# martenlienen/generative-turbulence

Hardware: AMD Instinct MI355X
Metric: U-Net fwd+bwd voxels/sec (DDPM training step, 192x64x48x4) (higher is better)
Workload: dtype bf16

## Files before the change

### generative-turbulence_amd/csrc/tdx_conv3.h

```cpp
#pragma once
#include "tdx_common.h"

struct Conv3Geom {
    int B;
    int Xi, Yi, Zi;
    int Xo, Yo, Zo;
    int off;
};

bool conv3_mfma_supported(int C1, int C2, int Cout);
bool conv3_mfma_f32_supported(int C1, int C2, int Cout);
static inline int conv3_layout_kc(int dtype, int K, int N) {
    if (dtype == 1 || dtype == 3) return conv3_mfma_supported(K, 0, N) ? 16 : 0;
    return conv3_mfma_f32_supported(K, 0, N) ? 8 : 0;
}
static inline bool conv3_uses_mfma_layout(int dtype, int K, int N) { return (dtype == 1 || dtype == 3) && conv3_mfma_supported(K, 0, N); }
bool conv3_mfma_split_supported(int C1, int C2, int Cout);

struct Conv3Ext {
    int ld1, ld2;
    const void* init;
    bool init_shared;
};

struct Conv3Call {
    const void* x1; int C1;
    const void* x2; int C2;
    const void* wp;
    const float* bias;
    void* y;
    int B, X, Y, Z, N;
    bool zero_pad;
    double* gn_acc;
    void* d1; int D1; void* d2;
    const void* a1; const void* a2;
    hipStream_t st;
    int fmt;
    const Conv3Ext* ext;
    const int* slabs_beyond;
    bool hf() const { return fmt == TDX_F16; }
    Conv3Geom geom() const { return Conv3Geom{B, X, Y, Z, X, Y, Z, 0}; }
};

struct SmallGeom {
    int B;
    int Ev[3];
    int Es[3];
    int off;
    int clamp;
    int nbg;
    int xs;
    int gx;
    int Ix, Iy, Iz;
    int K, N;
    int per_split;
    int nsplit;
};
struct Conv3SmallPlan {
    SmallGeom g;
    size_t lds;
    int mtw;
};

struct Conv3Route {
    int fmt, family, status;
    int ring_depth;
    Conv3SmallPlan small;
};
Conv3Route conv3_route(int dtype, int impl, int C1, int C2, int N, int B, int X, int Y, int Z, bool data_gradient);

int conv3_mfma_launch(const Conv3Call& c);
int conv3_mfma_split_launch(const Conv3Call& c);
int conv3_mfma_f32_launch(const Conv3Call& c);
int conv3_direct_launch(const Conv3Call& c);
int conv3_fold_launch(const Conv3Call& c);

int conv3_ring_depth(int C1, int C2, int N, int B, int X, int Y, int Z, bool data_gradient);
int conv3_ring_launch(const Conv3Call& c, int depth);

bool conv3_small_plan(Conv3SmallPlan& p, int C1, int C2, int N, int B, int X, int Y, int Z, bool data_gradient, bool split);
int conv3_small_launch(const Conv3Call& c, const Conv3SmallPlan& p);

struct Conv3WgradCall {
    const void* x1; int C1;
    const void* x2; int C2;
    const void* dy;
    float* dwp;
    float* dbias;
    int B, X, Y, Z, Cout;
    hipStream_t st;
    float* slabs; int max_slabs; int* nslab;
    bool hf;
};
bool tdx_deterministic();
static inline float* conv3_wgrad_merge(const Conv3WgradCall& c, int& nsplit, int64_t& slab_stride) {
    if (tdx_deterministic() && c.slabs != nullptr && nsplit > c.max_slabs) nsplit = c.max_slabs > 0 ? c.max_slabs : 1;
    const bool use_slabs = c.slabs != nullptr && nsplit <= c.max_slabs;
    slab_stride = use_slabs ? (int64_t)27 * (c.C1 + c.C2) * c.Cout : 0;
    if (c.nslab) *c.nslab = use_slabs ? nsplit : 0;
    return use_slabs ? c.slabs : c.dwp;
}
// ... 30 lines not shown
```

### generative-turbulence_amd/csrc/tdx_conv3_entry.hip

```cpp
#include "tdx_common.h"
#include "tdx_conv3.h"
#include <stdlib.h>
#include <algorithm>

int tdx_persistent_cus() {
    const char* env = getenv("TDX_PERSISTENT_CUS");
    int n = env ? atoi(env) : 256;
    n = n < 8 ? 8 : (n > 256 ? 256 : n);
    return n & ~7;
}
static void* g_scratch = nullptr;
static size_t g_scratch_bytes = 0;
void* tdx_scratch_ptr() { return g_scratch; }
size_t tdx_scratch_bytes() { return g_scratch_bytes; }
extern "C" int tdx_set_scratch(void* ptr, size_t bytes) {
    if (ptr != nullptr && bytes < 64) return TDX_EINVAL;
    g_scratch = ptr;
    g_scratch_bytes = ptr ? bytes : 0;
    return TDX_OK;
}

Conv3Route conv3_route(int dtype, int impl, int C1, int C2, int N, int B, int X, int Y, int Z, bool data_gradient) {
    Conv3Route r;
    r.fmt = dtype; r.family = TDX_KERNEL_DIRECT; r.status = TDX_OK; r.ring_depth = 0;
// ... 90 lines not shown
    if (!conv3_mfma_supported(C1, 0, Cout)) return TDX_ESHAPE;
    const bool det = tdx_deterministic();
    const Conv3Ext ext = {ld1, 0, init, init_shared != 0};
    Conv3Call c = conv3_fwd_call(x1, C1, nullptr, 0, wf, bias, y, B, X, Y, Z, Cout, dtype, stream);
    c.ext = &ext;
    c.gn_acc = (stats && !det) ? (double*)gn_workspace : nullptr;
    if (c.gn_acc && !clean) {
        int e = tdx_zero_async(c.gn_acc, (size_t)TDX_GN_REPLICAS * B * Cout * 2 * sizeof(double), c.st);
        if (e != TDX_OK) return e;
    }
    int rc = conv3_mfma_launch(c);
    if (rc != TDX_OK || !stats) return rc;
    if (det) return gn_stats_launch(y, stats, B, (int64_t)X * Y * Z, Cout, G, eps, dtype, gn_workspace, clean, c.st);
    return gn_finalize_launch(c.gn_acc, stats, B, Cout, G, (int64_t)X * Y * Z, eps, TDX_GN_REPLICAS, c.st);
}

extern "C" size_t tdx_conv3_bwd_data_workspace_bytes(int B, int X, int Y, int Z, int Cin, int dtype, int impl) {
    (void)impl;
    const size_t padded = (size_t)B * (X + 2) * (Y + 2) * (Z + 2) * Cin * (tdx_is_h16(dtype) ? 2 : 4);
    const size_t shell = conv3_shell_buffer_bytes(B, X, Y, Z, Cin);
    return (padded > shell ? padded : shell) + 256;
}

static int conv3_bwd_data_impl(const void* dy, const void* wb, void* dx1, int C1, void* dx2, int C2, const void* add1,
                               const void* add2, int B, int X, int Y, int Z, int Cout, int dtype, int impl,
                               void* workspace, void* stream) {
    TDX_CHECK_ARG(dy && wb && dx1 && workspace && B > 0 && X > 0 && Y > 0 && Z > 0 && C1 > 0 && C2 >= 0 && Cout > 0);
    TDX_CHECK_ARG(C2 == 0 || dx2);
    const int Cin = C1 + C2;
    if ((C1 % 8) || (C2 % 8) || (Cout % 8)) return TDX_ESHAPE;
    const Conv3Route r = conv3_route(dtype, impl, Cout, 0, Cin, B, X, Y, Z, true);
    if (r.status != TDX_OK) return r.status;
    Conv3Call c = {};
    c.x1 = dy; c.C1 = Cout; c.wp = wb;
    c.B = B; c.X = X; c.Y = Y; c.Z = Z; c.N = Cin;
    c.zero_pad = true;
    c.d1 = dx1; c.D1 = C1; c.d2 = dx2; c.a1 = add1; c.a2 = add2;
    c.st = as_stream(stream); c.fmt = r.fmt;
    if (r.family == TDX_KERNEL_DIRECT) c.y = workspace;
    int rc = conv3_launch(c, r);
    if (rc != TDX_OK || r.family == TDX_KERNEL_SMALL) return rc;
    if (r.family == TDX_KERNEL_DIRECT) return conv3_fold_launch(c);
    const int shell_mode = r.fmt == TDX_F16 ? 3 : (r.fmt == TDX_F32_SPLIT ? 2 : (r.fmt == TDX_F32 ? 1 : 0));
    return conv3_shell_launch(dy, wb, dx1, C1, dx2, B, X, Y, Z, Cout, Cin, shell_mode, c.st, workspace);
}

extern "C" int tdx_conv3_bwd_data(const void* dy, const void* wb, void* dx1, int C1, void* dx2, int C2,
                                  int accumulate, int B, int X, int Y, int Z, int Cout, int dtype, int impl,
                                  void* workspace, void* stream) {
    return conv3_bwd_data_impl(dy, wb, dx1, C1, dx2, C2, accumulate ? dx1 : nullptr, accumulate ? dx2 : nullptr, B, X, Y, Z,
                               Cout, dtype, impl, workspace, stream);
}

extern "C" int tdx_conv3_bwd_data_add(const void* dy, const void* wb, void* dx1, int C1, void* dx2, int C2,
                                      const void* add1, const void* add2, int B, int X, int Y, int Z, int Cout, int dtype,
                                      int impl, void* workspace, void* stream) {
    return conv3_bwd_data_impl(dy, wb, dx1, C1, dx2, C2, add1, add2, B, X, Y, Z, Cout, dtype, impl, workspace, stream);
}

#define W3_MAX_SLABS 8
static int w3_slab_capacity(int Cin, int Cout) {
    const int64_t c = ((int64_t)1 << 19) / ((int64_t)Cin * Cout);
    return (int)(c < W3_MAX_SLABS ? W3_MAX_SLABS : (c > 512 ? 512 : c));
}
extern "C" size_t tdx_conv3_bwd_weight_workspace_bytes(int Cin, int Cout, int impl) {
    (void)impl;
    return (size_t)(1 + w3_slab_capacity(Cin, Cout)) * 27 * Cin * Cout * sizeof(float) + (size_t)Cout * sizeof(float) + 512;
}

struct Conv3WgradRoute {
    int (*launch)(const Conv3WgradCall&);
    bool f32;
    int status;
};
static Conv3WgradRoute conv3_wgrad_route(int dtype, int impl, int C1, int C2, int Cout) {
    if (dtype == TDX_F32 && impl == TDX_CONV_SPLIT && conv3_wgrad_mfma_split_supported(C1, C2, Cout))
        return {conv3_wgrad_mfma_split_launch, true, TDX_OK};
    if (dtype == TDX_F32 && impl != TDX_CONV_DIRECT && conv3_wgrad_mfma_f32_supported(C1, C2, Cout))
        return {conv3_wgrad_mfma_f32_launch, true, TDX_OK};
    if (impl == TDX_CONV_MFMA || (impl == TDX_CONV_AUTO && tdx_is_h16(dtype) && conv3_wgrad_mfma_supported(C1, C2, Cout))) {
// ... 45 lines not shown
```

### generative-turbulence_amd/csrc/tdx_conv3_ring.hip

```cpp
#include "tdx_common.h"
#include "tdx_conv3.h"
#include "tdx_conv3_epilogue.h"
#include <algorithm>

#define RG_HY 10
#define RG_SZ 12
#define RG_SZ4 6
#define RG_WSLOTS 3
#define RG_WAVES 8
#define RG_STEPS 14
#ifndef RG_DEFAULT_LOADERS
#define RG_DEFAULT_LOADERS 1
#endif

struct RingArgs {
    const bf16* x1; const bf16* x2; int C1, C2;
    const bf16* wp; const float* bias; bf16* y;
    int B, X, Y, Z, Cout;
    int nbx, nby, nbz, ntn;
    double* gn_acc;
    bf16* d1; bf16* d2; int D1; const bf16* a1; const bf16* a2;
    const void* zeros;
    unsigned long long* stamps;
};

__device__ __forceinline__ void rg_dma_off(const void* sbase, unsigned voff, unsigned lds) {
    lds = __builtin_amdgcn_readfirstlane(lds);
    unsigned keep;
    asm volatile("s_mov_b32 %0, m0\n\ts_mov_b32 m0, %3\n\ts_nop 0\n\tglobal_load_lds_dwordx4 %1, %2\n\ts_mov_b32 m0, %0"
                 : "=&s"(keep) : "v"(voff), "s"(sbase), "s"(lds) : "memory");
}
#define RG_VMCNT(n) asm volatile("s_waitcnt vmcnt(%0)" ::"n"(n) : "memory")

#ifdef RG_STAMPS
#define RG_NSTAMP 64
#define RG_T()                                                                                        \
    do {                                                                                              \
        if (ord >= RG_STAMP_B0 && ord < RG_STAMP_B0 + 2) {                                            \
            const unsigned long long t_ = __builtin_amdgcn_s_memtime();                               \
            if (lane == 0 && nst < RG_NSTAMP) sStamp[wave * RG_NSTAMP + nst] = t_;                    \
            ++nst;                                                                                    \
        }                                                                                             \
    } while (0)
#else
#define RG_T() do { } while (0)
#endif
// ... 4 lines not shown
    static constexpr int BN = NT * 32;
    static constexpr int MT = 4 / NT;
    static constexpr int XP = Z4 ? MT : MT / 2;
    static constexpr int BX = 8 * XP;
    static constexpr int BZ = Z4 ? 4 : 8;
    static constexpr int HZ = BZ + 2;
    static constexpr int SZ = Z4 ? RG_SZ4 : RG_SZ;
    static constexpr int ENT = Z4 ? (BX + 2) / 2 * RG_HY * RG_SZ
                                  : (BX + 2) * RG_HY * SZ;
    static constexpr int APIECES = (ENT + 63) / 64;
    static constexpr int ABUF = APIECES * 1024;
    static constexpr int BPW = (APIECES + IW - 1) / IW;
    static constexpr int WPIECES = 28 * BN * 16 / 1024;
    static constexpr int WSLOT = WPIECES * 1024;
    static constexpr int WPW = (WPIECES + IW - 1) / IW;
    static constexpr int TILE = 32 * BN * 2;
    static constexpr int CH = BN / 8;
    static constexpr int VPI = 64 / CH;
    static constexpr int NST = MT * (32 / VPI);
    static constexpr size_t LDS = (size_t)2 * ABUF + (size_t)RG_WSLOTS * WSLOT + (size_t)RG_WAVES * TILE + 1024  +
                                  64  + BN * 4  + (size_t)RG_WAVES * BN * 2 * 4 ;
};

template <int NT, bool ZP, int LW, bool HF, bool Z4>
__global__ void __launch_bounds__(512 + 64 * LW, LW ? 3 : 2) conv3_ring_kernel(RingArgs A) {
    typedef RingShape<NT, LW, Z4> S;
    typedef H16<HF> H;
    typedef typename H::T HT;
    constexpr int BN = S::BN, MT = S::MT, XP = S::XP, BPW = S::BPW, WPW = S::WPW, CH = S::CH, VPI = S::VPI, NST = S::NST;
    static_assert(LW > 0 || BPW + WPW < RG_STEPS, "one DMA instruction per K step");
    extern __shared__ __attribute__((aligned(1024))) unsigned char smem[];
    unsigned char* sA = smem;
    unsigned char* sW = sA + 2 * S::ABUF;
    unsigned char* sT = sW + RG_WSLOTS * S::WSLOT;
    unsigned char* sD = sT + RG_WAVES * S::TILE;
    unsigned char* sZ = sD + 1024;
    float* sBias = reinterpret_cast<float*>(sZ + 64);
    float* sRed = sBias + BN;
    const unsigned lds0 = (unsigned)(size_t)(__attribute__((address_space(3))) const void*)smem;
    const unsigned ldsA = lds0, ldsW = lds0 + 2 * S::ABUF, ldsD = ldsW + RG_WSLOTS * S::WSLOT + RG_WAVES * S::TILE;

    const int tid = threadIdx.x, lane = tid & 63;
    const int wave = __builtin_amdgcn_readfirstlane(tid >> 6);
    const int r = lane & 31, hh = lane >> 5;
    const bool loader = LW > 0 && wave >= RG_WAVES;
    const int iw = LW ? wave - RG_WAVES : wave;
#ifdef RG_STAMPS
    unsigned long long* sStamp = reinterpret_cast<unsigned long long*>(NT == 2 ? sRed : sRed + RG_WAVES * BN * 2);
    int nst = 0;
#endif

    const int hw = blockIdx.x, xcd = hw & 7, slot = hw >> 3;
    const int ntile = slot % A.ntn, kx = slot / A.ntn, KX = (int)(gridDim.x >> 3) / A.ntn;
    const int nbricks = A.B * A.nbx * A.nby * A.nbz;
    const int lo = xcd * (nbricks >> 3) + min(xcd, nbricks & 7), hi = lo + (nbricks >> 3) + (xcd < (nbricks & 7) ? 1 : 0);
    const int nmine = hi - lo > kx ? (hi - lo - kx + KX - 1) / KX : 0;
    if (nmine == 0) return;
    const int n0 = ntile * BN;
    const int Cin = A.C1 + A.C2, nun = Cin >> 3;
    const int YZ = A.Y * A.Z, V = A.X * YZ;

    if (tid < BN) sBias[tid] = A.bias ? A.bias[n0 + tid] : 0.f;
    if (tid < 16) reinterpret_cast<unsigned*>(sZ)[tid] = 0u;
    lds_barrier();

    int hxyz[BPW];
#pragma unroll
    for (int i = 0; i < BPW; ++i) {
        const int pi = min(max(iw, 0) * BPW + i, S::APIECES - 1);
        const int e = min(pi * 64 + lane, S::ENT - 1);
        int hx, hy, hz;
        if (Z4) {
            const int xp = e / (RG_HY * RG_SZ), rem = e - xp * (RG_HY * RG_SZ), q = rem % RG_SZ;
            hy = rem / RG_SZ; hx = 2 * xp + q / RG_SZ4; hz = q % RG_SZ4;
        } else {
            hx = e / (RG_HY * S::SZ);
            const int rem = e - hx * (RG_HY * S::SZ);
            hy = rem / S::SZ; hz = min(rem - hy * S::SZ, S::HZ - 1);
        }
        hxyz[i] = hx | (hy << 8) | (hz << 16);
    }
    unsigned wlane[WPW];
#pragma unroll
    for (int j = 0; j < WPW; ++j) {
        const int pj = min(max(iw, 0) * WPW + j, S::WPIECES - 1);
        const int e = pj * 64 + lane;
// ... 138 lines not shown
#endif
        }
        RG_VMCNT(0);
        return;
    }
    bool stores_behind = false;

    f32x16 acc[NT][MT];

    for (int ord = 0; ord < nmine; ++ord) {
        int b, o0, o1, o2;
        brick_coords(ord, b, o0, o1, o2);
#pragma unroll
        for (int nt = 0; nt < NT; ++nt)
#pragma unroll
            for (int j = 0; j < 4; ++j) {
                const float4 bv = *reinterpret_cast<const float4*>(sBias + nt * 32 + 8 * j + 4 * hh);
#pragma unroll
                for (int mt = 0; mt < MT; ++mt) {
                    acc[nt][mt][4 * j] = bv.x; acc[nt][mt][4 * j + 1] = bv.y; acc[nt][mt][4 * j + 2] = bv.z; acc[nt][mt][4 * j + 3] = bv.w;
                }
            }

        for (int c8 = 0; c8 < nun; ++c8, ++u) {
            RG_T();
            if (LW == 0) { if (stores_behind) RG_VMCNT(WPW + NST); else RG_VMCNT(WPW); }
            stores_behind = false;
            RG_T();
            lds_barrier();
            RG_T();

            const unsigned char* bufA = sA + (u & 1) * S::ABUF;
            const unsigned char* slotW = sW + (u % RG_WSLOTS) * S::WSLOT;
            const unsigned char* xa[MT];
#pragma unroll
            for (int mt = 0; mt < MT; ++mt) xa[mt] = bufA + a_h[mt];

            bf16x8 xf[3][MT], wf[3][NT];
            auto read_frags = [&](int p, int fb) {
#pragma unroll
                for (int mt = 0; mt < MT; ++mt) {
                    const unsigned char* src = xa[mt] + xo[Z4 ? (mt & 1) : 0][p];
                    if (p == RG_STEPS - 1) src = hh ? sZ : src;
                    xf[fb][mt] = *reinterpret_cast<const bf16x8*>(src);
                }
#pragma unroll
                for (int nt = 0; nt < NT; ++nt) wf[fb][nt] = *reinterpret_cast<const bf16x8*>(slotW + p * (2 * BN * 16) + b_off[nt]);
// ... 10 lines not shown
#pragma unroll
                for (int nt = 0; nt < NT; ++nt)
#pragma unroll
                    for (int mt = 0; mt < MT; ++mt)
                        acc[nt][mt] = H::mfma(wf[p % 3][nt], xf[p % 3][mt], acc[nt][mt]);
                if (p + 2 < RG_STEPS) {
#pragma unroll
                    for (int k = 0; k < 4; ++k) {
                        __builtin_amdgcn_sched_group_barrier(0x008, 1, 0);
                        if (k < MT + NT) __builtin_amdgcn_sched_group_barrier(0x100, 1, 0);
                    }
                } else {
                    __builtin_amdgcn_sched_group_barrier(0x008, 4, 0);
                }
#if !defined(RG_ABL) || !(RG_ABL & 1)
                if (LW == 0 && p < BPW) issue_brick_piece(qs, (u + 1) & 1, p);
                if (LW == 0 && p >= BPW && p < BPW + WPW) issue_weight_piece(ws, uw % RG_WSLOTS, p - BPW);
#endif
                if (LW == 0 && p == BPW + WPW) {
                    ++uw;
                    if (++ws == nun) ws = 0;
                    if (++qs == nun) { qs = 0; ++qb; plan_brick(qb); }
                }
            }
        }

        RG_T();
        unsigned char* tile = sT + wave * S::TILE;
        const int last_b = b;
#pragma unroll
        for (int mt = 0; mt < MT; ++mt) {
            const int vw = ly * S::BZ + lz;
#pragma unroll
            for (int nt = 0; nt < NT; ++nt)
#pragma unroll
                for (int j = 0; j < 4; ++j) {
                    const int ch = nt * 32 + 8 * j + 4 * hh;
                    const unsigned lo2 = H::pack2(acc[nt][mt][4 * j], acc[nt][mt][4 * j + 1]);
                    const unsigned hi2 = H::pack2(acc[nt][mt][4 * j + 2], acc[nt][mt][4 * j + 3]);
                    *reinterpret_cast<uint2*>(tile + conv3_tile_addr16<BN>(vw, ch >> 3) + (ch & 7) * 2) = make_uint2(lo2, hi2);
                }
#pragma unroll
            for (int i = 0; i < 32 / VPI; ++i) {
                const int v = lane / CH + VPI * i, cidx = lane % CH;
                const int c0 = o0 + (Z4 ? wave * XP + mt : wave * XP + mt / 2);
                const int c1 = o1 + (Z4 ? (v >> 2) : 4 * (mt % 2) + (v >> 3)), c2 = o2 + (Z4 ? (v & 3) : (v & 7));
// ... 75 lines not shown
int conv3_ring_depth(int C1, int C2, int N, int B, int X, int Y, int Z, bool data_gradient) {
    if (data_gradient && (tdx_scratch_ptr() == nullptr || tdx_scratch_bytes() < 16)) return 0;
    return ring_brick_depth(C1, C2, N, B, X, Y, Z);
}
static bool ring_z8_supported(int C1, int C2, int Cout, int B, int X, int Y, int Z, int mode) {
    const int NT = Cout % 64 == 0 ? 2 : 1, bx = NT == 2 ? 8 : 16;
    if (X < bx || Y < 8 || Z < 8 || (X % bx) > 2 || (Y % 8) > 2 || (Z % 8) > 2) return false;
    const char* rag = getenv("TDX_RING_RAGGED");
    if (rag && atoi(rag) == 0 && ((X % bx) || (Y % 8) || (Z % 8))) return false;
    const int ntn = Cout / (32 * NT);
    if (ntn > tdx_persistent_cus() / 8) return false;
    if ((int64_t)X * Y * Z * 1024 >= (1ll << 31)) return false;
    if (mode == 2) return true;
    if (NT == 1 && std::max(C1, C2) > 32) return false;
    const int64_t nb = (int64_t)B * (X / bx) * (Y / 8) * (Z / 8);
    const char* mi = getenv("TDX_RING_MIN_ITEMS");
    return nb * ntn >= (mi ? atoi(mi) : 3 * 256);
}

#ifdef RG_STAMPS
static unsigned long long* rg_stamp_buffer = nullptr;
#endif

template <int NT, bool ZP, int LW, bool HF, bool Z4 = false>
static int ring_go(const RingArgs& a, hipStream_t st) {
    size_t lds = RingShape<NT, LW, Z4>::LDS;
#ifdef RG_STAMPS
    if (NT == 1) lds += (size_t)RG_WAVES * RG_NSTAMP * 8;
#endif
    const int px = tdx_persistent_cus() / 8, grid = 8 * (px - px % a.ntn);
    return tdx_launch_lds<conv3_ring_kernel<NT, ZP, LW, HF, Z4>>(dim3(grid), dim3(512 + 64 * LW), lds, st, a);
}

int conv3_ring_launch(const Conv3Call& c, int depth) {
    if ((depth != 4 && depth != 8) || !tdx_is_h16(c.fmt)) return TDX_EINVAL;
    if (c.zero_pad && (tdx_scratch_ptr() == nullptr || tdx_scratch_bytes() < 16)) return TDX_EINVAL;
    const int X = c.X, Y = c.Y, Z = c.Z;
    const bool zero_pad = c.zero_pad, hf = c.hf();
    hipStream_t st = c.st;
    const int NT = c.N % 64 == 0 ? 2 : 1;
    const int bxr = (NT == 2 ? 8 : 16) * (depth == 4 ? 2 : 1);
    RingArgs a;
    a.x1 = (const bf16*)c.x1; a.x2 = (const bf16*)c.x2; a.C1 = c.C1; a.C2 = c.C2;
    a.wp = (const bf16*)c.wp; a.bias = c.bias; a.y = (bf16*)c.y;
    a.B = c.B; a.X = X; a.Y = Y; a.Z = Z; a.Cout = c.N;
    a.nbx = X / bxr; a.nby = Y / 8; a.nbz = Z / depth; a.ntn = c.N / (32 * NT);
    a.gn_acc = c.gn_acc;
    a.d1 = (bf16*)c.d1; a.d2 = (bf16*)c.d2; a.D1 = c.D1; a.a1 = (const bf16*)c.a1; a.a2 = (const bf16*)c.a2;
    a.zeros = tdx_scratch_ptr();
    a.stamps = nullptr;
#ifdef RG_STAMPS
    a.stamps = rg_stamp_buffer;
#endif
    const char* env = getenv("TDX_RING_LOADERS");
    const bool lw = env ? atoi(env) != 0 : RG_DEFAULT_LOADERS;
    int rc = TDX_OK;
    if (depth == 4)
        TDX_DISPATCH_BOOL(NT == 2, WIDE, TDX_DISPATCH_BOOL(zero_pad, ZP, TDX_DISPATCH_H16(hf,
            rc = ring_go<WIDE ? 2 : 1, ZP, 4, HF, true>(a, st))));
    else if (hf || lw)
        TDX_DISPATCH_BOOL(NT == 2, WIDE, TDX_DISPATCH_BOOL(zero_pad, ZP, TDX_DISPATCH_H16(hf,
            rc = ring_go<WIDE ? 2 : 1, ZP, 4, HF>(a, st))));
    else
        TDX_DISPATCH_BOOL(NT == 2, WIDE, TDX_DISPATCH_BOOL(zero_pad, ZP, rc = ring_go<WIDE ? 2 : 1, ZP, 0, false>(a, st)));
    if (rc != TDX_OK || ((X % bxr) == 0 && (Y % 8) == 0 && (Z % depth) == 0)) return rc;
    const int beyond[3] = {X - X % bxr, Y - Y % 8, Z - Z % depth};
    Conv3Call rest = c;
    rest.slabs_beyond = beyond;
    return conv3_mfma_launch(rest);
}

extern "C" int tdx_conv3_uses_ring(int C1, int C2, int Cout, int B, int X, int Y, int Z) {
    return ring_brick_depth(C1, C2, Cout, B, X, Y, Z) != 0 ? 1 : 0;
}
extern "C" int tdx_conv3_ring_brick_depth(int C1, int C2, int Cout, int B, int X, int Y, int Z) {
    return ring_brick_depth(C1, C2, Cout, B, X, Y, Z);
}
```

### generative-turbulence_amd/turbdiff_amd/_lib.py

```python

from __future__ import annotations

import ctypes as C
import os
import threading
from pathlib import Path

import torch

_HERE = Path(__file__).resolve().parent
LIB_PATH = Path(os.environ.get("TDX_LIB", _HERE / "libtdx_hip.so"))

F32, BF16 = 0, 1
F16 = 3
CONV_AUTO, CONV_DIRECT, CONV_MFMA, CONV_SPLIT = 0, 1, 2, 3
F32_SPLIT = 2
WS_CLEAN = 0x100
ACT_NONE, ACT_SILU, ACT_GELU, ACT_RELU, ACT_SOFTPLUS, ACT_TANH = range(6)

_vp, _i, _i64, _u64, _f, _sz = C.c_void_p, C.c_int, C.c_int64, C.c_uint64, C.c_float, C.c_size_t

SIGNATURES = {
    "tdx_version": (_i, []),
    "tdx_arch": (C.c_char_p, []),
    "tdx_set_scratch": (_i, [_vp, _sz]),
    "tdx_ncv_to_nvc": (_i, [_vp, _vp, _i, _i, _i64, _i, _i, _vp]),
    "tdx_nvc_to_ncv": (_i, [_vp, _vp, _i, _i, _i64, _i, _i, _vp]),
    "tdx_cast": (_i, [_vp, _vp, _i64, _i, _i, _vp]),
    "tdx_conv3_pack_weight": (_i, [_vp, _vp, _vp, _i, _i, _i, _vp]),
    "tdx_conv3_pack_weights": (_i, [_vp, _i, _i, _vp]),
    "tdx_transpose_many": (_i, [_vp, _i, _vp]),
    "tdx_conv3_fwd": (_i, [_vp, _i, _vp, _i, _vp, _vp, _vp, _i, _i, _i, _i, _i, _i, _i, _vp]),
    "tdx_conv3_uses_ring": (_i, [_i] * 7),
    "tdx_conv3_ring_brick_depth": (_i, [_i] * 7),
    "tdx_conv3_fwd_kernel": (_i, [_i] * 9),
    "tdx_conv3_fwd_gn": (_i, [_vp, _i, _vp, _i, _vp, _vp, _vp, _vp, _i, _f, _vp, _i, _i, _i, _i, _i, _i, _i, _vp]),
    "tdx_conv3_fwd_partial": (_i, [_vp, _i, _i, _vp, _vp, _vp, _i, _vp, _vp, _i, _f, _vp, _i, _i, _i, _i, _i, _i, _i, _vp]),
    "tdx_conv3_bwd_data_workspace_bytes": (_sz, [_i, _i, _i, _i, _i, _i, _i]),
    "tdx_conv3_bwd_data": (_i, [_vp, _vp, _vp, _i, _vp, _i, _i, _i, _i, _i, _i, _i, _i, _i, _vp, _vp]),
    "tdx_conv3_bwd_data_add": (_i, [_vp, _vp, _vp, _i, _vp, _i, _vp, _vp, _i, _i, _i, _i, _i, _i, _i, _vp, _vp]),
    "tdx_conv3_bwd_weight_workspace_bytes": (_sz, [_i, _i, _i]),
    "tdx_conv3_bwd_weight": (_i, [_vp, _i, _vp, _i, _vp, _vp, _vp, _i, _i, _i, _i, _i, _i, _i, _vp, _vp]),
    "tdx_conv1_fwd": (_i, [_vp, _i, _vp, _i, _vp, _i, _vp, _vp, _vp, _i64, _i, _i, _vp]),
    "tdx_conv1_fwd_gn": (_i, [_vp, _i, _vp, _i, _vp, _i, _vp, _vp, _vp, _vp, _vp, _i, _vp, _i, _i64, _i, _i, _vp]),
    "tdx_conv1_bwd_weight": (_i, [_vp, _i, _vp, _i, _vp, _i, _vp, _i64, _i, _vp]),
    "tdx_conv1_bwd_weight_oc": (_i, [_vp, _i, _vp, _i, _vp, _i, _vp, _i, _i64, _i, _vp]),
    "tdx_encode_fwd": (_i, [_vp, _i, _vp, _vp, _vp, _i, _vp, _vp, _vp, _i, _i64, _i, _i, _vp]),
    "tdx_encode_bwd": (_i, [_vp, _vp, _i, _vp, _i, _vp, _vp, _vp, _vp, _vp, _vp, _i, _i64, _i, _i, _vp]),
    "tdx_decode_fwd": (_i, [_vp, _vp, _vp, _vp, _i, _i64, _i, _i, _i, _vp]),
    "tdx_decode_bwd": (_i, [_vp, _vp, _vp, _vp, _vp, _vp, _i, _i64, _i, _i, _i, _vp]),
    "tdx_gn_workspace_bytes": (_sz, [_i, _i]),
    "tdx_gn_stats": (_i, [_vp, _vp, _i, _i64, _i, _i, _f, _i, _vp, _vp]),
    "tdx_gn_apply": (_i, [_vp, _vp, _vp, _vp, _vp, _vp, _vp, _vp, _i, _i64, _i, _i, _i, _i, _vp]),
    "tdx_gn_apply_decode": (_i, [_vp, _vp, _vp, _vp, _vp, _vp, _vp, _vp, _i, _i64, _i, _i, _i, _i, _vp]),
    "tdx_gn_apply_encoded": (_i, [_vp, _vp, _vp, _vp, _vp, _i, _vp, _vp, _vp, _i, _vp, _vp, _vp, _i, _i64, _i, _i, _i, _vp]),
    "tdx_gn_apply_decode_act": (_i, [_vp, _vp, _vp, _vp, _vp, _vp, _vp, _vp, _i, _i64, _i, _i, _i, _i, _i, _vp]),
    "tdx_gn_apply_encoded_act": (_i, [_vp, _vp, _vp, _vp, _vp, _i, _vp, _vp, _vp, _i, _vp, _vp, _vp, _i, _i64, _i, _i, _i, _i, _vp]),
    "tdx_gn_bwd": (_i, [_vp] * 12 + [_i, _i64, _i, _i, _i, _i, _vp, _vp]),
    "tdx_bn_workspace_bytes": (_sz, [_i64, _i]),
    "tdx_bn_stats": (_i, [_vp, _vp, _vp, _i64, _i, _f, _i, _vp, _vp]),
    "tdx_bn_apply": (_i, [_vp, _vp, _vp, _vp, _vp, _i64, _vp, _i64, _i, _f, _i, _vp]),
    "tdx_bn_bwd": (_i, [_vp] * 8 + [_i64, _i, _f, _i, _i, _vp, _vp]),
    "tdx_flow_decompose_workspace_bytes": (_sz, [_i] * 7),
# ... 83 lines not shown
        if not LIB_PATH.exists():
            raise RuntimeError(
                f"{LIB_PATH} not found: the HIP kernels have not been built. "
                "Run `python -c 'import __graft_entry__ as g; g.build()'` (or `make -C generative-turbulence_amd/csrc`)."
            )
        lib = C.CDLL(str(LIB_PATH))
        lax = "TDX_LIB" in os.environ and os.environ.get("TDX_LIB_LAX") == "1"
        for name, (res, args) in SIGNATURES.items():
            if lax and not hasattr(lib, name):
                continue
            fn = getattr(lib, name)
            fn.restype = res
            fn.argtypes = args
        _lib = lib
    return _lib


_SCRATCH: "OrderedDict" = None
_ACTIVE = None
SCRATCH_BYTES = int(os.environ.get("TDX_SCRATCH_MB", "96")) << 20
SCRATCH_SMALL_BYTES = 4096
SCRATCH_MAX_ARENAS = int(os.environ.get("TDX_SCRATCH_MAX_ARENAS", "6"))
ARENA_USERS = {"tdx_conv3_fwd", "tdx_conv3_fwd_gn", "tdx_conv3_fwd_partial", "tdx_conv3_bwd_data", "tdx_conv3_bwd_data_add",
               "tdx_conv3_bwd_weight", "tdx_attn_fwd"}
DET_ARENA_USERS = {"tdx_conv1_bwd_weight", "tdx_conv1_bwd_weight_oc", "tdx_encode_bwd", "tdx_decode_bwd", "tdx_gn_stats"}


def deterministic() -> bool:
    return os.environ.get("TDX_DETERMINISTIC", "0") not in ("", "0")


_LAUNCH_LOCK = threading.RLock()
_SMALL_STREAMS = set()


def declare_zero_block_only(stream) -> None:
    _SMALL_STREAMS.add((stream.device.index, stream.cuda_stream))


def ensure_scratch(device=None) -> None:
    global _SCRATCH, _ACTIVE
    if _SCRATCH is None:
        from collections import OrderedDict

        _SCRATCH = OrderedDict()
    idx = torch.cuda.current_device() if device is None else torch.device(device).index
    idx = torch.cuda.current_device() if idx is None else idx
# ... 181 lines not shown
```

### generative-turbulence_amd/turbdiff_amd/ops.py

```python

from __future__ import annotations

import weakref

import os

import torch
from torch.autograd.function import once_differentiable

from . import _lib as L


def _ws(nbytes: int, device) -> torch.Tensor:
    return torch.empty(max(int(nbytes), 16), dtype=torch.uint8, device=device)


_CLEAN = {}
WS_CLEAN = 0 if os.environ.get("TDX_WS_CLEAN", "1") == "0" else L.WS_CLEAN


def _clean_ws(nbytes: int, device, tag=None) -> torch.Tensor:
    if not WS_CLEAN:
        return _ws(nbytes, device)
    key = (device, L.stream(device.index), int(nbytes), tag)
# ... 31 lines not shown

def _conv3_fwd(x1, C1, x2, C2, wf, bias, grid, Cout, code, impl, st, gn=None, ws=None, real=None, timed=True):
    B, X, Y, Z = grid
    y = x1.new_empty((B, X, Y, Z, Cout))
    work = 54.0 * (real or (C1 + C2)) * Cout * B * X * Y * Z if timed else 0.0
    meta = (lambda: L.conv3_fwd_meta(C1, C2, Cout, B, X, Y, Z, x1.dtype, real)) if timed else None
    if gn is None:
        L.call("tdx_conv3_fwd", L.ptr(x1), C1, L.ptr(x2), C2, L.ptr(wf), L.ptr(bias), L.ptr(y), B, X, Y, Z, Cout, code, impl, st,
               work=work, meta=meta)
        return y
    groups, eps = gn
    stats = x1.new_empty((B, groups, 2), dtype=torch.float32)
    if ws is None:
        ws = _gn_ws(B, Cout, x1.device, clean=True)
    L.call("tdx_conv3_fwd_gn", L.ptr(x1), C1, L.ptr(x2), C2, L.ptr(wf), L.ptr(bias), L.ptr(y), L.ptr(stats), groups, float(eps),
           L.ptr(ws), B, X, Y, Z, Cout, code, impl | WS_CLEAN, st, work=work, meta=meta)
    return y, stats


def _conv3_bwd_data_ws(grid, Cin, code, impl, dev):
    return _ws(L.query("tdx_conv3_bwd_data_workspace_bytes", *grid, Cin, code, impl), dev)


def _conv3_bwd_data(gy, wb, x1, C1, x2, C2, grid, Cout, code, impl, st, ws=None, add=None, real=None):
    B, X, Y, Z = grid
    gx1, gx2 = torch.empty_like(x1), None if x2 is None else torch.empty_like(x2)
    if ws is None:
        ws = _conv3_bwd_data_ws(grid, C1 + C2, code, impl, gy.device)
    work = 54.0 * (real or (C1 + C2)) * Cout * B * X * Y * Z
    if add is None:
        L.call("tdx_conv3_bwd_data", L.ptr(gy), L.ptr(wb), L.ptr(gx1), C1, L.ptr(gx2), C2, 0, B, X, Y, Z, Cout, code, impl,
               L.ptr(ws), st, work=work)
    else:
        L.call("tdx_conv3_bwd_data_add", L.ptr(gy), L.ptr(wb), L.ptr(gx1), C1, L.ptr(gx2), C2, L.ptr(add), None, B, X, Y, Z,
               Cout, code, impl, L.ptr(ws), st, work=work)
    return gx1, gx2


def _conv3_wgrad_out(wshape, has_bias, dev):
    return (torch.empty(wshape, dtype=torch.float32, device=dev),
            torch.empty(wshape[0], dtype=torch.float32, device=dev) if has_bias else None)


def _conv3_wgrad_ws(Cin, Cout, impl, dev):
    return _clean_ws(L.query("tdx_conv3_bwd_weight_workspace_bytes", Cin, Cout, impl), dev, ("w3", Cin, Cout))


def _conv3_wgrad(x1, C1, x2, C2, gy, gw, gb, grid, Cout, code, impl, ws, st, real=None):
    B, X, Y, Z = grid
    L.call("tdx_conv3_bwd_weight", L.ptr(x1), C1, L.ptr(x2), C2, L.ptr(gy), L.ptr(gw), L.ptr(gb), B, X, Y, Z, Cout, code,
           impl | WS_CLEAN, L.ptr(ws), st, work=54.0 * (real or (C1 + C2)) * Cout * B * X * Y * Z)


def _conv1_fwd(x1, C1, x2, C2, w, ldw, col, bias, add, lead, rows, Cout, code, st):
    y = x1.new_empty((*lead, Cout))
    L.call("tdx_conv1_fwd", L.ptr(x1), C1, L.ptr(x2), C2, L.ptr(w) + 4 * col, ldw, L.ptr(bias), L.ptr(add), L.ptr(y), rows, Cout,
           code, st)
    return y

# ... 1083 lines not shown
        side.run(lambda: _conv3_wgrad(a1, Cout, None, 0, dh2, dw2, db2, grid, Cout, code, impl, wws2, L.stream()), a1, dh2, dw2, db2)
        dws = _conv3_bwd_data_ws(grid, max(Cin, Cout, Cc), code, impl, dev)
        da1, _ = _conv3_bwd_data(dh2, wb2, a1, Cout, None, 0, grid, Cout, code, impl, st, dws)
        del dh2
        dfilm = torch.empty((2, B, Cout), dtype=torch.float32, device=dev)
        dh1, dg1, dbe1 = _gn_bwd(h1, da1, st1, g1, be1, scale, shift, dfilm[0], dfilm[1], B, V, Cout, groups, act, code, st, gws)
        del da1
        dw1, db1 = _conv3_wgrad_out(w1s, hb1, dev)
        if xc is not None:
            real = ctx.xc_real
            side.run(lambda: _conv3_wgrad(xc, Cc, None, 0, dh1, dw1, db1, grid, Cout, code, impl, wws1, L.stream(), real),
                     xc, dh1, dw1, db1)
            dxc = None
            if ctx.needs_input_grad[16]:
                dxc, _ = _conv3_bwd_data(dh1, wb1, xc, Cc, None, 0, grid, Cout, code, impl, st, dws, real=real)
            side.join()
            return (gy, None, dfilm, dw1, db1, dg1, dbe1, dw2, db2, dg2, dbe2, None, None, None, None, None, dxc, None, None,
                    None, None)
        side.run(lambda: _conv3_wgrad(x1, C1, x2, C2, dh1, dw1, db1, grid, Cout, code, impl, wws1, L.stream()),
                 x1, x2, dh1, dw1, db1)
        dwr = dbr = None
        if wr2 is None:
            gx1, gx2 = _conv3_bwd_data(dh1, wb1, x1, C1, None, 0, grid, Cout, code, impl, st, dws, add=gy)
        else:
            t1, t2 = _conv3_bwd_data(dh1, wb1, x1, C1, x2, C2, grid, Cout, code, impl, st, dws)
            gx1 = _conv1_fwd(gy, Cout, None, 0, wr2, Cin, 0, None, t1, grid, B * V, C1, code, st)
            gx2 = None if x2 is None else _conv1_fwd(gy, Cout, None, 0, wr2, Cin, C1, None, t2, grid, B * V, C2, code, st)
            dwr, dbr = _conv1_weight_grad(x1, C1, x2, C2, gy, Cout, hbr, B * V, code, st)
            dwr = dwr.view(wrs)
        side.join()
        return (gx1, gx2, dfilm, dw1, db1, dg1, dbe1, dw2, db2, dg2, dbe2, dwr, dbr, None, None, None, None, None, None, None, None)


def resnet_block(x1, x2, scale, shift, conv1_wb, norm1_wb, conv2_wb, norm2_wb, skip_wb, groups, eps=1e-5, partial=None,
                 conv1_input=None, conv1_real_channels=None, film=None, skip_encoded=None, decode_wb=None, act=ACT_SILU):
    wr, br = skip_wb if skip_wb is not None else (None, None)
    if act not in (ACT_SILU, ACT_GELU, ACT_RELU, ACT_SOFTPLUS, ACT_TANH):
        raise ValueError(f"resnet_block: act must be one of the TDX_ACT_* activation codes 1..5, got {act!r}")
    assert decode_wb is None or not torch.is_grad_enabled(), "decode_wb: inference only (the block output is not kept)"
    assert partial is None or not torch.is_grad_enabled(), "partial: inference only (the backward needs the full conv)"
    enc = None
    if skip_encoded is not None:
        assert x1 is skip_encoded.standin and conv1_input is not None and skip_wb is None and x2 is None
        enc = skip_encoded.operands
    if film is None:
        B, Cout = x1.shape[0], conv1_wb[0].shape[0]
        film = torch.stack((scale.reshape(B, Cout).float(), shift.reshape(B, Cout).float()))
    return _ResnetBlock.apply(x1, x2, film, conv1_wb[0], conv1_wb[1], norm1_wb[0], norm1_wb[1], conv2_wb[0],
                              conv2_wb[1], norm2_wb[0], norm2_wb[1], wr, br, groups, eps, partial, conv1_input,
                              conv1_real_channels, enc, decode_wb, int(act))
# ... 107 lines not shown
```

### include/tdx.h

```cpp
#ifndef TDX_H
#define TDX_H

#include <stddef.h>
#include <stdint.h>

#ifdef __cplusplus
extern "C" {
#endif

#define TDX_F32 0
#define TDX_BF16 1

#define TDX_OK 0
#define TDX_EINVAL (-1)
#define TDX_ESHAPE (-2)
#define TDX_EDTYPE (-3)

#define TDX_CONV_AUTO 0
#define TDX_CONV_DIRECT 1
#define TDX_CONV_MFMA 2
#define TDX_CONV_SPLIT 3
#define TDX_F32_SPLIT 2
#define TDX_F16 3
#define TDX_WS_CLEAN 0x100
// ... 27 lines not shown
int tdx_conv3_uses_ring(int C1, int C2, int Cout, int B, int X, int Y, int Z);
int tdx_conv3_ring_brick_depth(int C1, int C2, int Cout, int B, int X, int Y, int Z);
#define TDX_KERNEL_DIRECT 0
#define TDX_KERNEL_BRICK 1
#define TDX_KERNEL_SMALL 2
#define TDX_KERNEL_RING 3
int tdx_conv3_fwd_kernel(int C1, int C2, int Cout, int B, int X, int Y, int Z, int dtype, int impl);

int tdx_conv3_fwd_gn(const void* x1, int C1, const void* x2, int C2, const void* wf, const float* bias, void* y,
                     float* stats, int G, float eps, void* gn_workspace, int B, int X, int Y, int Z, int Cout,
                     int dtype, int impl, void* stream);

int tdx_conv3_fwd_partial(const void* x1, int C1, int ld1, const void* wf, const float* bias, const void* init,
                          int init_shared, void* y, float* stats, int G, float eps, void* gn_workspace, int B, int X,
                          int Y, int Z, int Cout, int dtype, int impl, void* stream);

size_t tdx_conv3_bwd_data_workspace_bytes(int B, int X, int Y, int Z, int Cin, int dtype, int impl);
int tdx_conv3_bwd_data(const void* dy, const void* wb, void* dx1, int C1, void* dx2, int C2, int accumulate,
                       int B, int X, int Y, int Z, int Cout, int dtype, int impl, void* workspace, void* stream);

int tdx_conv3_bwd_data_add(const void* dy, const void* wb, void* dx1, int C1, void* dx2, int C2, const void* add1,
                           const void* add2, int B, int X, int Y, int Z, int Cout, int dtype, int impl,
                           void* workspace, void* stream);

size_t tdx_conv3_bwd_weight_workspace_bytes(int Cin, int Cout, int impl);
int tdx_conv3_bwd_weight(const void* x1, int C1, const void* x2, int C2, const void* dy, float* dw, float* dbias,
                         int B, int X, int Y, int Z, int Cout, int dtype, int impl, void* workspace, void* stream);

int tdx_conv1_fwd(const void* x1, int C1, const void* x2, int C2, const float* w, int ldw, const float* bias,
                  const void* add, void* y, int64_t rows, int Cout, int dtype, void* stream);
int tdx_conv1_fwd_gn(const void* x1, int C1, const void* x2, int C2, const float* w, int ldw, const float* bias,
                     const void* h, const float* stats, const float* gamma, const float* beta, int groups, void* y,
                     int B, int64_t V, int Cout, int dtype, void* stream);
int tdx_conv1_bwd_weight(const void* x, int Cin, const void* dy, int Cout, float* dw, int ldw, float* dbias,
                         int64_t rows, int dtype, void* stream);
int tdx_conv1_bwd_weight_oc(const void* x, int Cin, const void* dy, int Cout, float* dw, int ldw, float* dbias,
                            int accumulate, int64_t rows, int dtype, void* stream);

int tdx_encode_fwd(const float* x, int Fx, const float* wx, const float* bx, const float* c, int Fc, const float* wc,
                   const float* bc, void* y, int B, int64_t V, int D, int dtype, void* stream);
int tdx_encode_bwd(const void* dy, const float* x, int Fx, const float* c, int Fc, const float* wc, float* dwx,
                   float* dbx, float* dwc, float* dbc, float* dc, int B, int64_t V, int D, int dtype, void* stream);
int tdx_decode_fwd(const void* h, const float* w, const float* bias, float* y, int B, int64_t V, int D, int F, int dtype,
                   void* stream);
int tdx_decode_bwd(const float* dy, const void* h, const float* w, void* dh, float* dw, float* db, int B, int64_t V, int D,
                   int F, int dtype, void* stream);
// ... 228 lines not shown
```

Baseline: 168.5 million.

## Fuse 1x1 skip-projection data gradient into ring conv3 backward-data kernel

```diff
diff --git a/generative-turbulence_amd/csrc/tdx_conv3.h b/generative-turbulence_amd/csrc/tdx_conv3.h
--- a/generative-turbulence_amd/csrc/tdx_conv3.h
+++ b/generative-turbulence_amd/csrc/tdx_conv3.h
@@ -34,6 +34,7 @@
     double* gn_acc;
     void* d1; int D1; void* d2;
     const void* a1; const void* a2;
+    const void* skip_x; const float* skip_w;
     hipStream_t st;
     int fmt;
     const Conv3Ext* ext;
@@ -77,6 +78,7 @@
 
 int conv3_ring_depth(int C1, int C2, int N, int B, int X, int Y, int Z, bool data_gradient);
 int conv3_ring_launch(const Conv3Call& c, int depth);
+bool conv3_ring_skip_supported(int fmt, int depth, int K, int N, int X, int Y, int Z);
 
 bool conv3_small_plan(Conv3SmallPlan& p, int C1, int C2, int N, int B, int X, int Y, int Z, bool data_gradient, bool split);
 int conv3_small_launch(const Conv3Call& c, const Conv3SmallPlan& p);
diff --git a/generative-turbulence_amd/csrc/tdx_conv3_entry.hip b/generative-turbulence_amd/csrc/tdx_conv3_entry.hip
--- a/generative-turbulence_amd/csrc/tdx_conv3_entry.hip
+++ b/generative-turbulence_amd/csrc/tdx_conv3_entry.hip
@@ -136,16 +136,21 @@
     return (padded > shell ? padded : shell) + 256;
 }
 
+static bool conv3_skip_routed(const Conv3Route& r, int Cin, int Cout, int X, int Y, int Z) {
+    return r.status == TDX_OK && r.family == TDX_KERNEL_RING && conv3_ring_skip_supported(r.fmt, r.ring_depth, Cout, Cin, X, Y, Z);
+}
 static int conv3_bwd_data_impl(const void* dy, const void* wb, void* dx1, int C1, void* dx2, int C2, const void* add1,
                                const void* add2, int B, int X, int Y, int Z, int Cout, int dtype, int impl,
-                               void* workspace, void* stream) {
+                               void* workspace, void* stream, const void* skip_dy = nullptr, const float* skip_w = nullptr) {
     TDX_CHECK_ARG(dy && wb && dx1 && workspace && B > 0 && X > 0 && Y > 0 && Z > 0 && C1 > 0 && C2 >= 0 && Cout > 0);
     TDX_CHECK_ARG(C2 == 0 || dx2);
     const int Cin = C1 + C2;
     if ((C1 % 8) || (C2 % 8) || (Cout % 8)) return TDX_ESHAPE;
     const Conv3Route r = conv3_route(dtype, impl, Cout, 0, Cin, B, X, Y, Z, true);
     if (r.status != TDX_OK) return r.status;
+    if (skip_dy != nullptr && !conv3_skip_routed(r, Cin, Cout, X, Y, Z)) return TDX_ESHAPE;
     Conv3Call c = {};
+    c.skip_x = skip_dy; c.skip_w = skip_w;
     c.x1 = dy; c.C1 = Cout; c.wp = wb;
     c.B = B; c.X = X; c.Y = Y; c.Z = Z; c.N = Cin;
     c.zero_pad = true;
@@ -170,6 +175,19 @@
                                       const void* add1, const void* add2, int B, int X, int Y, int Z, int Cout, int dtype,
                                       int impl, void* workspace, void* stream) {
     return conv3_bwd_data_impl(dy, wb, dx1, C1, dx2, C2, add1, add2, B, X, Y, Z, Cout, dtype, impl, workspace, stream);
+}
+
+extern "C" int tdx_conv3_bwd_data_skip_supported(int C1, int C2, int Cout, int B, int X, int Y, int Z, int dtype, int impl) {
+    if (B <= 0 || X <= 0 || Y <= 0 || Z <= 0 || C1 <= 0 || C2 < 0 || Cout <= 0 || (C1 % 8) || (C2 % 8) || (Cout % 8)) return 0;
+    return conv3_skip_routed(conv3_route(dtype, impl, Cout, 0, C1 + C2, B, X, Y, Z, true), C1 + C2, Cout, X, Y, Z) ? 1 : 0;
+}
+
+extern "C" int tdx_conv3_bwd_data_skip(const void* dy, const void* wb, void* dx1, int C1, void* dx2, int C2, const void* skip_dy,
+                                       const float* skip_w, int B, int X, int Y, int Z, int Cout, int dtype, int impl,
+                                       void* workspace, void* stream) {
+    TDX_CHECK_ARG(skip_dy && skip_w);
+    return conv3_bwd_data_impl(dy, wb, dx1, C1, dx2, C2, nullptr, nullptr, B, X, Y, Z, Cout, dtype, impl, workspace, stream,
+                               skip_dy, skip_w);
 }
 
 #define W3_MAX_SLABS 8
diff --git a/generative-turbulence_amd/csrc/tdx_conv3_ring.hip b/generative-turbulence_amd/csrc/tdx_conv3_ring.hip
--- a/generative-turbulence_amd/csrc/tdx_conv3_ring.hip
+++ b/generative-turbulence_amd/csrc/tdx_conv3_ring.hip
@@ -22,6 +22,7 @@
     bf16* d1; bf16* d2; int D1; const bf16* a1; const bf16* a2;
     const void* zeros;
     unsigned long long* stamps;
+    const bf16* skx; int skC; const float* skw; int skN;
 };
 
 __device__ __forceinline__ void rg_dma_off(const void* sbase, unsigned voff, unsigned lds) {
@@ -72,8 +73,10 @@
                                   64  + BN * 4  + (size_t)RG_WAVES * BN * 2 * 4 ;
 };
 
-template <int NT, bool ZP, int LW, bool HF, bool Z4>
+template <int NT, bool ZP, int LW, bool HF, bool Z4, int SK = 0>
 __global__ void __launch_bounds__(512 + 64 * LW, LW ? 3 : 2) conv3_ring_kernel(RingArgs A) {
+    static_assert(SK == 0 || (ZP && LW > 0 && !Z4 && 2 * SK * (NT * 32) * 16 == RG_WAVES * (NT * 32) * 2 * 4),
+                  "skip term: data gradient, loader form, 8-deep bricks, wr fills exactly the statistics scratch");
     typedef RingShape<NT, LW, Z4> S;
     typedef H16<HF> H;
     typedef typename H::T HT;
@@ -112,6 +115,15 @@
 
     if (tid < BN) sBias[tid] = A.bias ? A.bias[n0 + tid] : 0.f;
     if (tid < 16) reinterpret_cast<unsigned*>(sZ)[tid] = 0u;
+    if (SK > 0 && tid < 2 * SK * BN) {
+        const int kg = tid / BN, c = tid % BN;
+        const float* wsrc = A.skw + (size_t)(8 * kg) * A.skN + n0 + c;
+        float wv[8];
+#pragma unroll
+        for (int j = 0; j < 8; ++j) wv[j] = wsrc[(size_t)j * A.skN];
+        reinterpret_cast<uint4*>(sRed)[tid] =
+            make_uint4(H::pack2(wv[0], wv[1]), H::pack2(wv[2], wv[3]), H::pack2(wv[4], wv[5]), H::pack2(wv[6], wv[7]));
+    }
     lds_barrier();
 
     int hxyz[BPW];
@@ -296,7 +308,17 @@
                 }
             }
 
+        uint4 skf[SK > 0 ? SK : 1][MT];
         for (int c8 = 0; c8 < nun; ++c8, ++u) {
+            if (SK > 0 && c8 == nun - 1) {
+#pragma unroll
+                for (int mt = 0; mt < MT; ++mt) {
+                    const int64_t sv = (int64_t)b * V + (o0 + wave * XP + mt / 2) * YZ + (o1 + 4 * (mt % 2) + ly) * A.Z + o2 + lz;
+#pragma unroll
+                    for (int s = 0; s < SK; ++s)
+                        skf[s][mt] = *reinterpret_cast<const uint4*>(A.skx + sv * A.skC + 16 * s + 8 * hh);
+                }
+            }
             RG_T();
             if (LW == 0) { if (stores_behind) RG_VMCNT(WPW + NST); else RG_VMCNT(WPW); }
             stores_behind = false;
@@ -353,6 +375,21 @@
                     if (++ws == nun) ws = 0;
                     if (++qs == nun) { qs = 0; ++qb; plan_brick(qb); }
                 }
+            }
+        }
+
+        if (SK > 0) {
+#pragma unroll
+            for (int s = 0; s < SK; ++s) {
+                bf16x8 wsk[NT];
+#pragma unroll
+                for (int nt = 0; nt < NT; ++nt)
+                    wsk[nt] = *reinterpret_cast<const bf16x8*>(reinterpret_cast<const unsigned char*>(sRed) + s * (2 * BN * 16) + b_off[nt]);
+#pragma unroll
+                for (int nt = 0; nt < NT; ++nt)
+#pragma unroll
+                    for (int mt = 0; mt < MT; ++mt)
+                        acc[nt][mt] = H::mfma(wsk[nt], __builtin_bit_cast(bf16x8, skf[s][mt]), acc[nt][mt]);
             }
         }
 
@@ -474,14 +511,26 @@
 static unsigned long long* rg_stamp_buffer = nullptr;
 #endif
 
-template <int NT, bool ZP, int LW, bool HF, bool Z4 = false>
+template <int NT, bool ZP, int LW, bool HF, bool Z4 = false, int SK = 0>
 static int ring_go(const RingArgs& a, hipStream_t st) {
     size_t lds = RingShape<NT, LW, Z4>::LDS;
 #ifdef RG_STAMPS
     if (NT == 1) lds += (size_t)RG_WAVES * RG_NSTAMP * 8;
 #endif
     const int px = tdx_persistent_cus() / 8, grid = 8 * (px - px % a.ntn);
-    return tdx_launch_lds<conv3_ring_kernel<NT, ZP, LW, HF, Z4>>(dim3(grid), dim3(512 + 64 * LW), lds, st, a);
+    return tdx_launch_lds<conv3_ring_kernel<NT, ZP, LW, HF, Z4, SK>>(dim3(grid), dim3(512 + 64 * LW), lds, st, a);
+}
+
+static bool ring_loader_form(bool hf) {
+    const char* env = getenv("TDX_RING_LOADERS");
+    return hf || (env ? atoi(env) != 0 : RG_DEFAULT_LOADERS);
+}
+bool conv3_ring_skip_supported(int fmt, int depth, int K, int N, int X, int Y, int Z) {
+    const char* env = getenv("TDX_SKIP_DGRAD_FUSE");
+    if (env && atoi(env) == 0) return false;
+    if (!tdx_is_h16(fmt) || depth != 8 || K != 32 || N <= 0 || (N % 64) != 0) return false;
+    if ((X % 8) || (Y % 8) || (Z % 8)) return false;
+    return ring_loader_form(fmt == TDX_F16);
 }
 
 int conv3_ring_launch(const Conv3Call& c, int depth) {
@@ -504,13 +553,24 @@
 #ifdef RG_STAMPS
     a.stamps = rg_stamp_buffer;
 #endif
-    const char* env = getenv("TDX_RING_LOADERS");
-    const bool lw = env ? atoi(env) != 0 : RG_DEFAULT_LOADERS;
+    a.skx = nullptr; a.skC = 0; a.skw = nullptr; a.skN = 0;
+    if (c.skip_x != nullptr || c.skip_w != nullptr) {
+#ifdef RG_STAMPS
+        return TDX_ESHAPE;
+#else
+        if (!c.skip_x || !c.skip_w || !zero_pad || c.C2 != 0 || !conv3_ring_skip_supported(c.fmt, depth, c.C1, c.N, X, Y, Z)) return TDX_ESHAPE;
+        a.skx = (const bf16*)c.skip_x; a.skC = c.C1; a.skw = c.skip_w; a.skN = c.N;
+        int rcs = TDX_OK;
+        TDX_DISPATCH_H16(hf, rcs = ring_go<2, true, 4, HF, false, 2>(a, st));
+        return rcs;
+#endif
+    }
+    const bool lw = ring_loader_form(hf);
     int rc = TDX_OK;
     if (depth == 4)
         TDX_DISPATCH_BOOL(NT == 2, WIDE, TDX_DISPATCH_BOOL(zero_pad, ZP, TDX_DISPATCH_H16(hf,
             rc = ring_go<WIDE ? 2 : 1, ZP, 4, HF, true>(a, st))));
-    else if (hf || lw)
+    else if (lw)
         TDX_DISPATCH_BOOL(NT == 2, WIDE, TDX_DISPATCH_BOOL(zero_pad, ZP, TDX_DISPATCH_H16(hf,
             rc = ring_go<WIDE ? 2 : 1, ZP, 4, HF>(a, st))));
     else
diff --git a/generative-turbulence_amd/turbdiff_amd/_lib.py b/generative-turbulence_amd/turbdiff_amd/_lib.py
--- a/generative-turbulence_amd/turbdiff_amd/_lib.py
+++ b/generative-turbulence_amd/turbdiff_amd/_lib.py
@@ -39,6 +39,8 @@
     "tdx_conv3_bwd_data_workspace_bytes": (_sz, [_i, _i, _i, _i, _i, _i, _i]),
     "tdx_conv3_bwd_data": (_i, [_vp, _vp, _vp, _i, _vp, _i, _i, _i, _i, _i, _i, _i, _i, _i, _vp, _vp]),
     "tdx_conv3_bwd_data_add": (_i, [_vp, _vp, _vp, _i, _vp, _i, _vp, _vp, _i, _i, _i, _i, _i, _i, _i, _vp, _vp]),
+    "tdx_conv3_bwd_data_skip_supported": (_i, [_i] * 9),
+    "tdx_conv3_bwd_data_skip": (_i, [_vp, _vp, _vp, _i, _vp, _i, _vp, _vp, _i, _i, _i, _i, _i, _i, _i, _vp, _vp]),
     "tdx_conv3_bwd_weight_workspace_bytes": (_sz, [_i, _i, _i]),
     "tdx_conv3_bwd_weight": (_i, [_vp, _i, _vp, _i, _vp, _vp, _vp, _i, _i, _i, _i, _i, _i, _i, _vp, _vp]),
     "tdx_conv1_fwd": (_i, [_vp, _i, _vp, _i, _vp, _i, _vp, _vp, _vp, _i64, _i, _i, _vp]),
@@ -168,7 +170,7 @@
 SCRATCH_SMALL_BYTES = 4096
 SCRATCH_MAX_ARENAS = int(os.environ.get("TDX_SCRATCH_MAX_ARENAS", "6"))
 ARENA_USERS = {"tdx_conv3_fwd", "tdx_conv3_fwd_gn", "tdx_conv3_fwd_partial", "tdx_conv3_bwd_data", "tdx_conv3_bwd_data_add",
-               "tdx_conv3_bwd_weight", "tdx_attn_fwd"}
+               "tdx_conv3_bwd_data_skip", "tdx_conv3_bwd_weight", "tdx_attn_fwd"}
 DET_ARENA_USERS = {"tdx_conv1_bwd_weight", "tdx_conv1_bwd_weight_oc", "tdx_encode_bwd", "tdx_decode_bwd", "tdx_gn_stats"}
 
 
diff --git a/generative-turbulence_amd/turbdiff_amd/ops.py b/generative-turbulence_amd/turbdiff_amd/ops.py
--- a/generative-turbulence_amd/turbdiff_amd/ops.py
+++ b/generative-turbulence_amd/turbdiff_amd/ops.py
@@ -77,19 +77,36 @@
     return _ws(L.query("tdx_conv3_bwd_data_workspace_bytes", *grid, Cin, code, impl), dev)
 
 
-def _conv3_bwd_data(gy, wb, x1, C1, x2, C2, grid, Cout, code, impl, st, ws=None, add=None, real=None):
+def _conv3_bwd_data(gy, wb, x1, C1, x2, C2, grid, Cout, code, impl, st, ws=None, add=None, real=None, skip=None):
     B, X, Y, Z = grid
     gx1, gx2 = torch.empty_like(x1), None if x2 is None else torch.empty_like(x2)
     if ws is None:
         ws = _conv3_bwd_data_ws(grid, C1 + C2, code, impl, gy.device)
     work = 54.0 * (real or (C1 + C2)) * Cout * B * X * Y * Z
-    if add is None:
+    if skip is not None:
+        sgy, sw = skip
+        L.call("tdx_conv3_bwd_data_skip", L.ptr(gy), L.ptr(wb), L.ptr(gx1), C1, L.ptr(gx2), C2, L.ptr(sgy), L.ptr(sw), B, X, Y, Z,
+               Cout, code, impl, L.ptr(ws), st, work=work + 2.0 * Cout * (C1 + C2) * B * X * Y * Z)
+    elif add is None:
         L.call("tdx_conv3_bwd_data", L.ptr(gy), L.ptr(wb), L.ptr(gx1), C1, L.ptr(gx2), C2, 0, B, X, Y, Z, Cout, code, impl,
                L.ptr(ws), st, work=work)
     else:
         L.call("tdx_conv3_bwd_data_add", L.ptr(gy), L.ptr(wb), L.ptr(gx1), C1, L.ptr(gx2), C2, L.ptr(add), None, B, X, Y, Z,
                Cout, code, impl, L.ptr(ws), st, work=work)
     return gx1, gx2
+
+
+def skip_dgrad_static(Cout, grid, dt, wdt=torch.float32):
+    _, X, Y, Z = grid
+    return dt in L.H16_DTYPES and wdt == torch.float32 and Cout == 32 and X % 8 == 0 and Y % 8 == 0 and Z % 8 == 0
+
+
+def _skip_dgrad_fused(C1, C2, Cout, grid, dt, wdt, code, impl):
+    if not skip_dgrad_static(Cout, grid, dt, wdt):
+        return False
+    with L._LAUNCH_LOCK:
+        L.ensure_scratch()
+        return L.query("tdx_conv3_bwd_data_skip_supported", C1, C2, Cout, *grid, code, impl) == 1
 
 
 def _conv3_wgrad_out(wshape, has_bias, dev):
@@ -1219,10 +1236,13 @@
         dwr = dbr = None
         if wr2 is None:
             gx1, gx2 = _conv3_bwd_data(dh1, wb1, x1, C1, None, 0, grid, Cout, code, impl, st, dws, add=gy)
+        elif _skip_dgrad_fused(C1, C2, Cout, grid, gy.dtype, wr2.dtype, code, impl):
+            gx1, gx2 = _conv3_bwd_data(dh1, wb1, x1, C1, x2, C2, grid, Cout, code, impl, st, dws, skip=(gy, wr2))
         else:
             t1, t2 = _conv3_bwd_data(dh1, wb1, x1, C1, x2, C2, grid, Cout, code, impl, st, dws)
             gx1 = _conv1_fwd(gy, Cout, None, 0, wr2, Cin, 0, None, t1, grid, B * V, C1, code, st)
             gx2 = None if x2 is None else _conv1_fwd(gy, Cout, None, 0, wr2, Cin, C1, None, t2, grid, B * V, C2, code, st)
+        if wr2 is not None:
             dwr, dbr = _conv1_weight_grad(x1, C1, x2, C2, gy, Cout, hbr, B * V, code, st)
             dwr = dwr.view(wrs)
         side.join()
diff --git a/include/tdx.h b/include/tdx.h
--- a/include/tdx.h
+++ b/include/tdx.h
@@ -73,6 +73,11 @@
 int tdx_conv3_bwd_data_add(const void* dy, const void* wb, void* dx1, int C1, void* dx2, int C2, const void* add1,
                            const void* add2, int B, int X, int Y, int Z, int Cout, int dtype, int impl,
                            void* workspace, void* stream);
+
+int tdx_conv3_bwd_data_skip_supported(int C1, int C2, int Cout, int B, int X, int Y, int Z, int dtype, int impl);
+int tdx_conv3_bwd_data_skip(const void* dy, const void* wb, void* dx1, int C1, void* dx2, int C2, const void* skip_dy,
+                            const float* skip_w, int B, int X, int Y, int Z, int Cout, int dtype, int impl,
+                            void* workspace, void* stream);
 
 size_t tdx_conv3_bwd_weight_workspace_bytes(int Cin, int Cout, int impl);
 int tdx_conv3_bwd_weight(const void* x1, int C1, const void* x2, int C2, const void* dy, float* dw, float* dbias,
```

New measurement: 172.3 million, median of 6. 1.02x the previous value.
